# datastryio/weaviate

Measured on AMD Instinct MI355X. Metric: batched 10-NN QPS at recall@10≥0.95, 1M×128-d L2, on 1/2/4/8 MI355X, higher is better.
Workload: dtype f32 (f16 MFMA keys certified by an error bound, f32 reference-order re-rank); 1 GPU; exact brute-force 10-NN, 1,000,000 x 128-d l2-squared, 10000-query batch (BASELINE configs[1]); N=1000000, dim=128, nq=10000, k=10, metric=l2-squared, mode=exact, split=corpus, parallelism=corpus sharded over 1 GPU(s) by id range

## Files before the change

weaviate_amd/csrc/wv_api.hip:

```cpp
#include <hip/hip_runtime.h>
#include <hipcub/hipcub.hpp>

#include <algorithm>
#include <array>
#include <atomic>
#include <chrono>
#include <cmath>
#include <cstdio>
#include <cstdlib>
#include <condition_variable>
#include <cstring>
#include <mutex>
#include <string>
#include <thread>
#include <vector>

#include "../../include/wvgpu.h"
#include "wv_device.h"

#include "wv_params.h"

extern "C" {
hipError_t wv_launch_bf_mfma(const wv::BfParams* p, hipStream_t s);
hipError_t wv_launch_bf_finalize(const wv::BfFinParams* p, hipStream_t s);
hipError_t wv_launch_bf_finalize_wide(const wv::BfFinParams* p, hipStream_t s);
hipError_t wv_launch_exact_scan(const wv::ScanParams* p, hipStream_t s);
hipError_t wv_launch_fb(const wv::FbParams* p, hipStream_t s);
hipError_t wv_launch_fbd(const int32_t* flags, int nq, const wv::FbParams* fb, hipStream_t s);
hipError_t wv_launch_fbd_mark(const int32_t* status, int nq, int32_t* flags, float* thr, const float* out_d,
                              const int32_t* out_n, int k, hipStream_t s);
hipError_t wv_launch_hnsw_stats(const uint32_t* counters, int nq, unsigned long long* acc, hipStream_t s);
hipError_t wv_launch_rownorm(const float* X, uint64_t N, int D, int ldx, float* norm2, unsigned int* maxbits,
                             hipStream_t s);
hipError_t wv_launch_normalize(const float* in, float* out, uint64_t n, int D, int ld, hipStream_t s);
hipError_t wv_launch_scale(const float* in, float* out, uint64_t n, float scale, hipStream_t s);
hipError_t wv_launch_qnorm(const float* Q, int nq, int D, int ldq, int metric, float* out, float* absmax_part,
                           hipStream_t s);
hipError_t wv_launch_hnsw(const wv::HnswParams* p, int waves_per_block, hipStream_t s);
hipError_t wv_launch_hnsw_wg(const wv::HnswParams* p, hipStream_t s);
hipError_t wv_launch_build_search(const wv::BuildParams* b, int waves_per_block, hipStream_t s);
hipError_t wv_launch_build_select(const wv::BuildParams* b, hipStream_t s);
hipError_t wv_launch_build_link(const wv::BuildParams* b, hipStream_t s);
int wv_hnsw_per_wave_words(int dpad, int efc, int sc, int vc_log2, int xs_log2);
int wv_hnsw_side_per_wave_words(int dpad, int side_rows, int vc_log2, int xs_log2);
int wv_hnsw_reg_per_wave_words(int dpad, int vc_log2);
hipError_t wv_launch_hnsw_side(const wv::HnswParams* p, int waves_per_block, int ev, hipStream_t s);
hipError_t wv_launch_sbd_scan(const wv::SbdParams* p, hipStream_t s);
hipError_t wv_sbd_sort(unsigned long long* keys, unsigned long long* tmp, const unsigned int* cnt, int nq, int cap,
                       int* offsets, void** scratch, size_t* scratch_cap, hipStream_t s);
hipError_t wv_launch_pq_encode(const float* X, int ldx, const uint64_t* ids, uint64_t n_rows, const wv::PqParams* pq,
                               uint8_t* codes, hipStream_t s);
hipError_t wv_launch_pq_scan(const wv::PqScanParams* p, hipStream_t s);
hipError_t wv_launch_split_rows(const float* in, int ld_in, const uint64_t* ids, uint64_t n, uint64_t n_valid, int D,
                                float scale, void* out, int ld_out, uint64_t out_row0, hipStream_t s);
hipError_t wv_launch_h16_rows(const float* in, int ld_in, const uint64_t* ids, uint64_t n, int D, int ns, float sign,
                              float scale, const unsigned int* scale_from_max, void* out, uint64_t out_row0,
                              unsigned int* res_max_bits, float* res_out, int wide_layout, hipStream_t s);
hipError_t wv_launch_h16_rows_gather(const float* in, int ld_in, const uint32_t* gather, uint64_t n, uint64_t n_pad,
                                     int D, int ns, float scale, void* out, hipStream_t s);
hipError_t wv_launch_h16_compact_aux(const float* xnorm, const uint32_t* rowidx, uint64_t n, const uint32_t* n_dev,
                                     float* cxnorm, uint64_t* excl, uint64_t excl_words, hipStream_t s);
hipError_t wv_launch_remap_ids(uint32_t* ids, int nq, int n_slots, int per_slot, int bq, uint64_t ntiles,
                               uint64_t units_per_block, const uint32_t* rowidx, uint64_t n_rows, const uint32_t* n_dev,
                               hipStream_t s);
hipError_t wv_launch_absmax(const float* in, int ld, uint64_t n, int D, unsigned int* max_bits, hipStream_t s);
hipError_t wv_launch_h16_qscale(const float* part, int nparts, unsigned int* max_bits, float bsign, float* qscale,
                                hipStream_t s);
hipError_t wv_launch_h16_xns(const float* xnorm, uint64_t n, float sx, const float* qscale, float* xns, hipStream_t s);
hipError_t wv_launch_bf_h16(const wv::H16Params* p, int ns, int seed, hipStream_t s);
hipError_t wv_launch_bf_h16w(const wv::H16Params* p, hipStream_t s);
// ... 470 lines not shown
    return WV_OK;
}

int run_h16(wv_index* ix, const float* d_q, int nq, int k, const uint64_t* d_allow, uint64_t allow_nbits, uint64_t N,
            uint64_t* d_out_ids, float* d_out_d, int32_t* d_out_n, hipStream_t s, std::vector<int32_t>& fails,
            const uint32_t* rowidx = nullptr, const uint32_t* n_dev = nullptr) {
    const int ns = ix->h16_ns;
    const bool wd = ix->h16_wide;
    const int wg_per_cu = 1;
    const int tile_rows = wd ? wv::HW_BN : wv::H_BN, bq = wd ? wv::HW_BQ : 512;
    const int seed_prod = wd ? wv::HW_PROD : wv::H_PROD;
    const int prod = seed_prod;
    const int kp = wv::BF_KP;
    const uint64_t ntl = (N + tile_rows - 1) / tile_rows;
    const uint64_t words = ntl * (uint64_t)(tile_rows / 64);
    const uint64_t* allow = d_allow;
    if (d_allow && (allow_nbits + 63) / 64 < words) {
        HIP_TRY(ix->allow_pad.ensure(words * 8));
        HIP_TRY(hipMemsetAsync(ix->allow_pad.p, 0, words * 8, s));
        if (allow_nbits)
            HIP_TRY(hipMemcpyAsync(ix->allow_pad.p, d_allow, (allow_nbits + 63) / 64 * 8, hipMemcpyDeviceToDevice, s));
        allow = ix->allow_pad.as<uint64_t>();
    }
    const int nqb = (nq + bq - 1) / bq;
    const size_t qbytes = (size_t)nqb * bq * ns * 16 * 2;
    HIP_TRY(ix->qimg16.ensure(qbytes));
    HIP_TRY(ix->qres.ensure((size_t)nq * 4));
    HIP_TRY(ix->tau.ensure((size_t)nq * 4));
    HIP_TRY(ix->gtau.ensure((size_t)nq * 4));
    HIP_TRY(ix->q_nrm2.ensure((size_t)nq * 4));
    HIP_TRY(ix->fail.ensure((size_t)nq * 4));
    HIP_TRY(ix->fail_thr.ensure((size_t)nq * 4));
    const float bsign = ix->metric == WV_L2_SQUARED ? -2.f : -1.f;
    HIP_TRY(ix->qmax_part.ensure((size_t)((nq + 3) / 4) * 4));
    HIP_TRY(wv_launch_qnorm(d_q, nq, ix->dim, ix->dpad, ix->metric, ix->q_nrm2.as<float>(), ix->qmax_part.as<float>(),
                            s));
    HIP_TRY(hipMemsetAsync(ix->qimg16.p, 0, qbytes, s));
    HIP_TRY(wv_launch_h16_qscale(ix->qmax_part.as<float>(), (nq + 3) / 4, ix->qmax.as<unsigned int>(), bsign,
                                 ix->qscale.as<float>(), s));
    HIP_TRY(wv_launch_h16_rows(d_q, ix->dpad, nullptr, nq, ix->dim, ns, bsign, 1.f, ix->qmax.as<unsigned int>(),
                               ix->qimg16.p, 0, nullptr, ix->qres.as<float>(), 0, s));
    const void* ximg = ix->ximg16.p;
    const float* xnorm = ix->xnorm.as<float>();
    const uint64_t* excl = ix->excl.as<uint64_t>();
    if (rowidx) {
        const uint64_t rows = ntl * tile_rows, ew = rows / 64 + 2;
        HIP_TRY(ix->cxnorm.ensure(rows * 4));
        HIP_TRY(ix->cexcl.ensure(ew * 8));
        HIP_TRY(hipMemsetAsync(ix->cxnorm.p, 0, rows * 4, s));
        if (!wd) {
            const size_t ib = rows * (size_t)ns * 16 * 2;
            HIP_TRY(ix->cimg16.ensure(ib));
            HIP_TRY(wv_launch_h16_rows_gather(ix->vecs.as<float>(), ix->ldx, rowidx, N, rows, ix->dim, ns, ix->h16_sx,
                                              ix->cimg16.p, s));
            ximg = ix->cimg16.p;
        }
        HIP_TRY(wv_launch_h16_compact_aux(ix->xnorm.as<float>(), rowidx, N, n_dev, ix->cxnorm.as<float>(),
                                          ix->cexcl.as<uint64_t>(), ew, s));
        xnorm = ix->cxnorm.as<float>();
        excl = ix->cexcl.as<uint64_t>();
        allow = nullptr;
    }
    if (ix->metric == WV_L2_SQUARED)
        HIP_TRY(wv_launch_h16_xns(xnorm, ntl * tile_rows, ix->h16_sx, ix->qscale.as<float>(), ix->xns.as<float>(), s));
    wv::H16Params hp{};
    hp.X = ximg;
    hp.rowidx = wd ? rowidx : nullptr;
    hp.Q = ix->qimg16.p;
    hp.xns = ix->xns.as<float>();
    hp.excl = excl;
    hp.allow = allow;
    hp.qscale = ix->qscale.as<float>();
    hp.sx = ix->h16_sx;
    hp.N = N;
    hp.nq = nq;
    hp.metric = ix->metric;
    hp.n_qblocks = nqb;
    hp.wide_rows = 128;
    hp.clean_tiles = wd ? 0 : rowidx ? N / wv::H_BN : allow ? 0 : std::min<uint64_t>(ix->clean_words, N / wv::H_BN);
    hp.locality = 1;
    wv::BfFinParams fp{};
    fp.X = ix->vecs.as<float>();
    fp.Q = d_q;
    fp.qnorm = ix->q_nrm2.as<float>();
    fp.xnorm_max = ix->maxnorm_host;
    fp.nq = nq;
    fp.D = ix->dim;
    fp.ldx = ix->ldx;
    fp.ldq = ix->dpad;
    fp.metric = ix->metric;
    fp.k = k;
    fp.id_base = ix->cfg.id_base;
    fp.out_ids = d_out_ids;
    fp.out_d = d_out_d;
    fp.out_n = d_out_n;
    fp.fail = ix->fail.as<int32_t>();
    fp.fail_thr = ix->fail_thr.as<float>();
// ... 79 lines not shown
        sp.bq = bq;
        sp.prod = seed_prod;
        if (seed_lists) {
            HIP_TRY(wv_launch_h16_seed(&sp, s));
            HIP_TRY(ix->seed_d.ensure((size_t)nq * ss.n_slots * prod * kp * 4));
            HIP_TRY(ix->seed_id.ensure((size_t)nq * ss.n_slots * prod * kp * 4));
            hp.ntiles = ss.ntiles;
            hp.ntiles_real = ss.ntiles;
            hp.units_per_block = ss.units_per_block;
            hp.n_slots = ss.n_slots;
            hp.tile_stride = 1;
            hp.tile_base = ntl_main;
            hp.tau = ix->tau.as<float>();
            hp.out_d = ix->seed_d.as<float>();
            hp.out_id = ix->seed_id.as<uint32_t>();
            HIP_TRY(wv_launch_bf_h16(&hp, ns, 0, s));
            hp.tile_base = 0;
            hp.tau = nullptr;
            sp.minima = ix->seed_d.as<float>();
            sp.ids = ix->seed_id.as<uint32_t>();
            sp.n_slots = ss.n_slots;
            sp.ntiles = ss.ntiles;
            sp.units_per_block = ss.units_per_block;
            sp.prod = prod * kp;
            sp.out_d = ix->cand_d.as<float>();
            sp.out_id = ix->cand_id.as<uint32_t>();
            sp.out_slots = out_slots;
            sp.out_ntiles = sch.ntiles;
            sp.out_upb = sch.units_per_block;
        }
        HIP_TRY(wv_launch_h16_seed(&sp, s));
        return WV_OK;
    };
    if (seed) {
        TREC(6);
        int mult = 4;
        if (const char* e = std::getenv("WV_H16_LIST_MULT")) mult = std::max(1, std::atoi(e));
        if (int rc = seed_minima(seed_lists ? mult * sample : sample)) return rc;
        TREC(7);
    }
    hp.ntiles = sch.ntiles;
    hp.ntiles_real = ntl_main;
    hp.out_slots = seed_lists ? out_slots : 0;
    hp.units_per_block = sch.units_per_block;
    hp.n_slots = sch.n_slots;
    hp.n_dev = n_dev;
    hp.tile_stride = 1;
    hp.tau = nullptr;
    if (!seed) HIP_TRY(hipMemsetAsync(ix->gtau.p, 0xFF, (size_t)nq * 4, s));
    hp.gtau = ix->gtau.as<unsigned int>();
    hp.kth = k <= (wd ? 2 * kp : prod * kp) && !seed && !std::getenv("WV_H16_NO_RUNNING")
                 ? k
                 : 0;
    if (xs_fits(sch)) {
        const size_t gb = (size_t)nq * 2 * sch.n_slots * 4;
        HIP_TRY(ix->gslot.ensure(gb));
        HIP_TRY(hipMemsetAsync(ix->gslot.p, 0x7F, gb, s));
        hp.gslot = ix->gslot.as<float>();
        hp.xslot = 1;
        hp.kth = k;
    }
    if (hp.kth) {
        HIP_TRY(ix->marg.ensure((size_t)nq * 4));
        HIP_TRY(wv_launch_h16_margin(ix->metric, ix->dim, ix->q_nrm2.as<float>(), ix->qres.as<float>(),
                                     ix->maxnorm_host, ix->h16_ex, ix->h16_sx, ix->qscale.as<float>(), nq,
                                     ix->marg.as<float>(), s));
        hp.marg = ix->marg.as<float>();
    }
    hp.out_d = ix->cand_d.as<float>();
    hp.out_id = ix->cand_id.as<uint32_t>();
    const bool rotate = !wd && nqb >= 2 && sch.ntiles == ntl_main;
    if (rotate) hp.locality |= 2;
    if (int rc = block_order(ix, (uint64_t)nqb, sch, s, &hp.block_order, rotate)) return rc;
    TREC(0);
    HIP_TRY(wd ? wv_launch_bf_h16w(&hp, s) : wv_launch_bf_h16(&hp, ns, 0, s));
    TREC(1);
    if (rowidx && wide)
        HIP_TRY(wv_launch_remap_ids(ix->cand_id.as<uint32_t>(), nq, sch.n_slots, prod * kp, bq, sch.ntiles,
                                    sch.units_per_block, rowidx, N, n_dev, s));
    if (rowidx && !wide) {
        fp.rowidx = rowidx;
        fp.rowidx_n = N;
        fp.rowidx_ndev = n_dev;
    }
    fp.cand_d = ix->cand_d.as<float>();
    fp.cand_id = ix->cand_id.as<uint32_t>();
    fp.n_slots = out_slots;
    fp.extra_slot = seed_lists ? 1 : 0;
    fp.ntiles = sch.ntiles;
    fp.units_per_block = sch.units_per_block;
    HIP_TRY(wv_launch_h16_gtau(ix->gtau.as<unsigned int>(), nq, ix->h16_sx, ix->qscale.as<float>(), ix->tau.as<float>(),
                               s));
    fp.tau_in = ix->tau.as<float>();
    TREC(2);
    HIP_TRY(wide ? wv_launch_bf_finalize_wide(&fp, s) : wv_launch_bf_finalize(&fp, s));
    TREC(3);
    (void)fails;
    return WV_OK;
}

int queue_fbd(wv_index* ix, const float* d_q, int nq, int k, const uint64_t* d_allow, uint64_t allow_nbits,
              uint64_t allow_stride, uint64_t* d_out_ids, float* d_out_d, int32_t* d_out_n, hipStream_t s) {
    const uint64_t N = ix->n_rows;
    HIP_TRY(ix->fbd_list.ensure((size_t)nq * 4));
    HIP_TRY(ix->fbd_nf.ensure(16));
    HIP_TRY(ix->fbd_over.ensure((size_t)nq * 4));
    HIP_TRY(ix->fbd_cd.ensure((size_t)nq * wv::FB_CAP * 4));
    HIP_TRY(ix->fbd_ci.ensure((size_t)nq * wv::FB_CAP * 4));
    HIP_TRY(ix->fbd_cn.ensure((size_t)nq * 4));
    HIP_TRY(ix->fbd_scr.ensure((size_t)wv::FBD_SCR * std::max<uint64_t>(N, 1) * 4));
    HIP_TRY(ix->stat_acc.ensure(48));
    wv::FbParams bp{};
    bp.X = ix->vecs.as<float>();
    bp.Q = d_q;
    bp.qidx = ix->fbd_list.as<int32_t>();
    bp.thr = ix->fail_thr.as<float>();
    bp.tomb = ix->excl.as<uint64_t>();
    bp.tomb_nbits = ix->capacity;
    bp.allow = d_allow;
    bp.allow_nbits = allow_nbits;
    bp.allow_stride = allow_stride;
    bp.N = N;
    bp.nf = nq;
    bp.D = ix->dim;
    bp.ldx = ix->ldx;
    bp.ldq = ix->dpad;
// ... 2222 lines not shown
```

weaviate_amd/csrc/wv_bf.hip:

```cpp
#include "wv_device.h"
#include "wv_params.h"
#include "wv_topk.h"

#include <float.h>

namespace wv {


typedef __bf16 bf16x8 __attribute__((ext_vector_type(8)));




__device__ __forceinline__ void list_insert(float (&ld)[BF_KP], uint32_t (&li)[BF_KP], float d, uint32_t id) {
#pragma unroll
    for (int i = 0; i < BF_KP; ++i) {
        const bool lt = key_less(d, id, ld[i], li[i]);
        const float td = ld[i];
        const uint32_t ti = li[i];
        ld[i] = lt ? d : ld[i];
        li[i] = lt ? id : li[i];
        d = lt ? td : d;
        id = lt ? ti : id;
    }
// ... 599 lines not shown
                if (hi == mi && hd == md && mi != WV_NIL) head++;
                if (lane == 0) { sd[r] = md; si[r] = mi; }
            }
        }
    }
    __builtin_amdgcn_wave_barrier();
    {
        const float dk = sd[FIN_KF - 1];
        const uint32_t ik = si[FIN_KF - 1];
        if (key_less(dk, ik, bound, bound_id)) { bound = dk; bound_id = ik; }
    }
    if (p.h16 && bound != FLT_MAX) bound *= 1.0f / (p.sx * p.qscale[0]);
    if (p.tau_in) bound = fminf(bound, p.tau_in[q]);

    for (int i = lane; i < ((p.D + 3) & ~3); i += 64) qv[i] = i < p.D ? p.Q[(size_t)q * p.ldq + i] : 0.f;
    __builtin_amdgcn_wave_barrier();

    int n_sel = 0;
    for (int j = 0; j < FIN_KF; ++j) n_sel += (si[j] != WV_NIL);
    __builtin_amdgcn_wave_barrier();
    if (p.rowidx) {
        const uint64_t nr = p.rowidx_ndev ? (uint64_t)*p.rowidx_ndev : p.rowidx_n;
        uint32_t v = WV_NIL;
        if (lane < FIN_KF && si[lane] != WV_NIL && si[lane] < nr) v = p.rowidx[si[lane]];
        const uint64_t vm = __ballot(v != WV_NIL);
        __builtin_amdgcn_wave_barrier();
        if (lane < FIN_KF) si[lane] = WV_NIL;
        __builtin_amdgcn_wave_barrier();
        if (v != WV_NIL) si[mbcnt64(vm)] = v;
        n_sel = __popcll(vm);
        if (lane < FIN_KF && lane >= n_sel) sd[lane] = FLT_MAX;
        __builtin_amdgcn_wave_barrier();
    }
    exact_dist_rows<METRIC, FIN_KF / 8>(qv, p.X, p.ldx, p.D, si, n_sel, sd, lane);
    __builtin_amdgcn_wave_barrier();
    float myd = FLT_MAX;
    uint32_t myi = WV_NIL;
    int rank = 0;
    if (lane < FIN_KF) {
        myd = sd[lane];
        myi = si[lane];
        const uint64_t mykey = fin_key(myd, myi);
        for (int j = 0; j < FIN_KF; ++j)
            rank += fin_key(sd[j], si[j]) < mykey;
    }
    __builtin_amdgcn_wave_barrier();
    const int k = p.k;
    int nvalid = 0;
    for (int j = 0; j < FIN_KF; ++j) nvalid += (si[j] != WV_NIL);
    if (lane < FIN_KF && myi != WV_NIL && rank < k && !p.tau_out) {
        p.out_ids[(size_t)q * k + rank] = p.id_base + myi;
        p.out_d[(size_t)q * k + rank] = myd;
    }
    float dk = -FLT_MAX;
    const int nk = nvalid < k ? nvalid : k;
    if (lane < FIN_KF && myi != WV_NIL && rank == nk - 1) dk = myd;
    for (int m = 32; m >= 1; m >>= 1) dk = fmaxf(dk, __shfl_xor(dk, m, 64));

    const float u = 5.9604645e-08f;
    const float D4 = (float)(p.D + 4);
    float eps, bfull;
    const float acc_f = p.split ? 12.f : 4.f;
    const float split_e = p.split ? 4.f * 1.52587890625e-05f : 0.f;
    if (METRIC == WV_METRIC_L2) {
        const float qn = sqrtf(p.qnorm[q]);
        const float s = qn + p.xnorm_max;
        eps = acc_f * D4 * u * s * s + 2.f * split_e * qn * p.xnorm_max;
        bfull = bound + p.qnorm[q];
    } else {
        const float qn = p.qnorm[q];
        eps = acc_f * D4 * u * qn * p.xnorm_max + 4.f * u + split_e * qn * p.xnorm_max;
        bfull = METRIC == WV_METRIC_DOT ? bound : 1.0f + bound;
    }
    eps *= 1.0001f;
    if (p.h16) eps = h16_eps(METRIC, p.D, p.qnorm[q], p.xnorm_max, p.ex_max, p.qres[q]);
    if (p.tau_out) {
        float tau = __builtin_inff();
        if (nvalid >= k && dk < FLT_MAX) {
            const float off = METRIC == WV_METRIC_L2 ? p.qnorm[q] : (METRIC == WV_METRIC_DOT ? 0.f : 1.0f);
            tau = dk - off + eps;
            tau += 4.f * u * (fabsf(dk) + fabsf(off) + eps) + 1e-3f * eps;
        }
        if (lane == 0) p.tau_out[q] = tau;
        return;
    }
    bool certified;
    if (nvalid < k) certified = bound == FLT_MAX;
    else certified = (bound == FLT_MAX) || (bfull - eps > dk);
    if (lane == 0) {
        p.out_n[q] = nk;
        p.fail[q] = certified ? 0 : 1;
        p.fail_thr[q] = nvalid < k ? __builtin_inff() : dk;
    }
}

template <bool FAST>
__global__ __launch_bounds__(64) void wv_bf_finalize_kernel(BfFinParams p) {
    extern __shared__ float qv[];
    const int dpad = (p.D + 3) & ~3;
    float* sd = qv + dpad;
    uint32_t* si = reinterpret_cast<uint32_t*>(sd + FIN_KF);
    float* kept_d = reinterpret_cast<float*>(si + FIN_KF);
    uint32_t* kept_i = reinterpret_cast<uint32_t*>(kept_d + 256);
    const int q = blockIdx.x;
    if (q >= p.nq) return;
    if (p.metric == WV_METRIC_L2) finalize_one<WV_METRIC_L2, FAST>(p, q, sd, si, qv, kept_d, kept_i);
    else if (p.metric == WV_METRIC_DOT) finalize_one<WV_METRIC_DOT, FAST>(p, q, sd, si, qv, kept_d, kept_i);
    else finalize_one<WV_METRIC_COSINE, FAST>(p, q, sd, si, qv, kept_d, kept_i);
// ... 530 lines not shown
    }
    if (norm == 0.f) {
        for (int i = 0; i < D; ++i) o[i] = 0.f;
        return;
    }
    const float nn = (float)sqrt((double)norm);
    for (int i = 0; i < D; ++i) o[i] = __fdiv_rn(v[i], nn);
}

__device__ __forceinline__ uint16_t bf16_rn(float v) {
    const uint32_t b = __float_as_uint(v);
    return (uint16_t)((b + 0x7FFFu + ((b >> 16) & 1u)) >> 16);
}
__global__ void wv_split_rows_kernel(const float* in, int ld_in, const uint64_t* ids, uint64_t n, uint64_t n_valid,
                                     int D, float scale, uint16_t* out, int ld_out, uint64_t out_row0) {
    const uint64_t t = (uint64_t)blockIdx.x * blockDim.x + threadIdx.x;
    const uint64_t r = t / (uint64_t)ld_out;
    const int k = (int)(t % (uint64_t)ld_out);
    if (r >= n) return;
    const uint64_t row = ids ? ids[r] : r;
    const float v = (k < D && r < n_valid) ? scale * in[row * ld_in + k] : 0.f;
    const uint16_t hi = bf16_rn(v);
    const uint16_t lo = bf16_rn(v - __uint_as_float((uint32_t)hi << 16));
    const uint64_t o = split_hi_index(out_row0 + row, k, ld_out / BF_BK);
    out[o] = hi;
    out[o + 512] = lo;
}

__global__ void wv_scale_rows_kernel(const float* in, float* out, uint64_t n, float s) {
    const uint64_t i = (uint64_t)blockIdx.x * blockDim.x + threadIdx.x;
    if (i < n) out[i] = s * in[i];
}

__global__ __launch_bounds__(256) void wv_qnorm_kernel(const float* Q, int nq, int D, int ldq, int metric, float* out,
                                                       float* absmax_part) {
    __shared__ float wmax[4];
    const int lane = threadIdx.x & 63, w = threadIdx.x >> 6;
    const int r = blockIdx.x * 4 + w;
    float s = 0.f, m = 0.f;
    if (r < nq) {
        const float* q = Q + (size_t)r * ldq;
        for (int i = lane; i < D; i += 64) {
            const float v = q[i];
            s = __builtin_fmaf(v, v, s);
            m = fmaxf(m, fabsf(v));
        }
    }
    for (int o = 32; o >= 1; o >>= 1) {
        s += __shfl_xor(s, o, 64);
        m = fmaxf(m, __shfl_xor(m, o, 64));
    }
    if (r < nq && lane == 0) out[r] = metric == WV_METRIC_L2 ? s : sqrtf(s * (1.0f + 1e-6f)) * (1.0f + 1e-6f);
    if (absmax_part) {
        if (lane == 0) wmax[w] = m;
        __syncthreads();
        if (threadIdx.x == 0) absmax_part[blockIdx.x] = fmaxf(fmaxf(wmax[0], wmax[1]), fmaxf(wmax[2], wmax[3]));
    }
}

}

extern "C" {

hipError_t wv_launch_bf_mfma(const wv::BfParams* p, hipStream_t s) {
    if (p->X == nullptr || p->Q == nullptr) return hipErrorInvalidValue;
    const uint64_t total = (uint64_t)p->n_qblocks * p->ntiles;
    const unsigned nb = (unsigned)((total + p->units_per_block - 1) / p->units_per_block);
    if (nb == 0) return hipSuccess;
    if (p->split) {
        const int nk = p->ldx / wv::BF_BK;
        if (p->ldx % wv::BF_BK || p->ldq != p->ldx || nk < 1 || nk > 4 || p->rowidx || p->allow_stride)
            return hipErrorInvalidValue;
        const bool l2 = p->metric == WV_METRIC_L2;
        const bool wide = p->bq == 2 * wv::BF_BQ;
        if (!wide && p->bq != wv::BF_BQ) return hipErrorInvalidValue;
        const size_t lds = (size_t)nk * (wide ? 32768 : 16384) + (wide ? 8 : 4) * 256;
#define WV_SPLIT_LAUNCH(NK)                                                                                   \
        if (wide) {                                                                                           \
            if (l2) hipLaunchKernelGGL((wv::wv_bf_split_kernel<NK, true, 4>), dim3(nb), dim3(512), lds, s, *p);  \
            else hipLaunchKernelGGL((wv::wv_bf_split_kernel<NK, false, 4>), dim3(nb), dim3(512), lds, s, *p);    \
        } else {                                                                                              \
            if (l2) hipLaunchKernelGGL((wv::wv_bf_split_kernel<NK, true, 2>), dim3(nb), dim3(256), lds, s, *p);  \
            else hipLaunchKernelGGL((wv::wv_bf_split_kernel<NK, false, 2>), dim3(nb), dim3(256), lds, s, *p);    \
        }
        switch (nk) {
// ... 95 lines not shown
hipError_t wv_launch_exact_scan(const wv::ScanParams* p, hipStream_t s) {
    uint64_t blocks = (p->N + 31) / 32;
    if (blocks > 8192) blocks = 8192;
    if (blocks == 0) blocks = 1;
    hipLaunchKernelGGL(wv::wv_exact_scan_kernel, dim3((unsigned)blocks), dim3(256), p->D * sizeof(float), s, *p);
    return hipGetLastError();
}

hipError_t wv_launch_rownorm(const float* X, uint64_t N, int D, int ldx, float* norm2, unsigned int* maxbits,
                             hipStream_t s) {
    if (N == 0) return hipSuccess;
    hipLaunchKernelGGL(wv::wv_rownorm_kernel, dim3((unsigned)((N + 255) / 256)), dim3(256), 0, s, X, N, D, ldx,
                       norm2, maxbits);
    return hipGetLastError();
}

hipError_t wv_launch_normalize(const float* in, float* out, uint64_t n, int D, int ld, hipStream_t s) {
    if (n == 0) return hipSuccess;
    hipLaunchKernelGGL(wv::wv_normalize_kernel, dim3((unsigned)((n + 255) / 256)), dim3(256), 0, s, in, out, n, D,
                       ld);
    return hipGetLastError();
}

hipError_t wv_launch_scale(const float* in, float* out, uint64_t n, float scale, hipStream_t s) {
    if (n == 0) return hipSuccess;
    hipLaunchKernelGGL(wv::wv_scale_rows_kernel, dim3((unsigned)((n + 255) / 256)), dim3(256), 0, s, in, out, n,
                       scale);
    return hipGetLastError();
}

hipError_t wv_launch_qnorm(const float* Q, int nq, int D, int ldq, int metric, float* out, float* absmax_part,
                           hipStream_t s) {
    if (nq == 0) return hipSuccess;
    hipLaunchKernelGGL(wv::wv_qnorm_kernel, dim3((nq + 3) / 4), dim3(256), 0, s, Q, nq, D, ldq, metric, out,
                       absmax_part);
    return hipGetLastError();
}

}
```

weaviate_amd/csrc/wv_h16.hip:

```cpp
#include "wv_device.h"
#include "wv_params.h"
#include "wv_topk.h"

#include <float.h>

#include "wv_h16_dev.h"

namespace wv {


constexpr bool min_steps_cover(int ns) {
    unsigned m = 0;
    for (int k = 0; k < ns; ++k) {
        if (k == 0) m |= 7u;
        else if (k <= 6) m |= 3u << (2 * k + 1);
        if (k == ns - 1)
            for (int r = ns <= 7 ? 2 * ns + 1 : 15; r < 16; ++r) m |= 1u << r;
    }
    return m == 0xFFFFu;
}

template <int NS, bool L2, bool SEED, bool XS = false>
__global__ __launch_bounds__(512, 1) void wv_bf_h16_kernel(H16Params p) {
    static_assert(min_steps_cover(NS), "the spread tile minima must cover all 16 keys of a half");
// ... 800 lines not shown
                    const float th = fminf(ld[BF_KP - 1], pt);
                    const float m = min16(A);
                    const bool x = m <= th;
                    if (__any(x)) {
                        WV_DBG_COUNT(3)
                        min_extract(m, x, A, pt, ld, li, rr);
                    }
                };
                xt(A0, l0d, l0i, pt0, rb);
                xt(B0, l0d, l0i, pt0, rb + 32);
                xt(A1, l1d, l1i, pt1, rb);
                xt(B1, l1d, l1i, pt1, rb + 32);
#endif
            }
            if (running && (tc < 8 || (tc & 3) == 3)) publish();
        }
        vm_wait(0);
        block_barrier();
        const int prod = rh * 2 + khalf;
        const size_t per_q = (size_t)p.n_slots * HW_PROD * BF_KP;
        if (jq0 < p.nq) {
            const size_t base = (size_t)jq0 * per_q + ((size_t)slot * HW_PROD + prod) * BF_KP;
#pragma unroll
            for (int i = 0; i < BF_KP; ++i) { p.out_d[base + i] = l0d[i]; p.out_id[base + i] = l0i[i]; }
        }
        if (jq1 < p.nq) {
            const size_t base = (size_t)jq1 * per_q + ((size_t)slot * HW_PROD + prod) * BF_KP;
#pragma unroll
            for (int i = 0; i < BF_KP; ++i) { p.out_d[base + i] = l1d[i]; p.out_id[base + i] = l1i[i]; }
        }
    }
}

__global__ __launch_bounds__(64) void wv_h16_seed_kernel(H16SeedParams p) {
    const int q = blockIdx.x;
    const int lane = threadIdx.x;
    if (q >= p.nq) return;
    const int prod = p.prod ? p.prod : H_PROD;
    const int n = bf_slots_of((uint64_t)(q / p.bq), p.ntiles, p.units_per_block) * prod;
    const float* m = p.minima + (size_t)q * p.n_slots * prod;
    const float inv_s = 1.0f / (p.sx * p.qscale[0]);
    float mk = __builtin_inff();
    if (p.ids) {
        const size_t off = (size_t)q * p.n_slots * prod;
        uint64_t kk[4];
#pragma unroll
        for (int j = 0; j < 4; ++j) {
            const int e = 64 * j + lane;
            const uint32_t id = e < n ? p.ids[off + e] : WV_NIL;
            kk[j] = fin_key(id != WV_NIL ? p.minima[off + e] : FLT_MAX, id);
        }
        bitonic256_wave(kk, lane);
        float d;
        uint32_t id;
        fin_unkey(kk[0], d, id);
        const float dk = __shfl(d, p.k - 1, 64);
        const uint32_t ik = (uint32_t)__shfl((int)id, p.k - 1, 64);
        if (ik != WV_NIL) mk = dk;
        const int os = bf_slots_of((uint64_t)(q / p.bq), p.out_ntiles, p.out_upb);
        const size_t ob = ((size_t)q * p.out_slots + os) * H_PROD * BF_KP;
        if (lane < H_PROD * BF_KP) {
            const size_t o = ob + (size_t)(lane & 1) * BF_KP + (lane >> 1);
            p.out_d[o] = d;
            p.out_id[o] = id;
        }
    } else if (n <= 256) {
        float v[4];
#pragma unroll
        for (int j = 0; j < 4; ++j) v[j] = 64 * j + lane < n ? m[64 * j + lane] : __builtin_inff();
#pragma unroll
        for (int kk = 2; kk <= 256; kk <<= 1) {
#pragma unroll
            for (int jj = kk >> 1; jj > 0; jj >>= 1) {
                if (jj >= 64) {
                    const int mm = jj >> 6;
#pragma unroll
                    for (int j = 0; j < 4; ++j) {
                        const int pj = j ^ mm;
                        if (pj <= j) continue;
                        const bool up = ((64 * j + lane) & kk) == 0;
                        const float lo = fminf(v[j], v[pj]), hi = fmaxf(v[j], v[pj]);
                        v[j] = up ? lo : hi;
                        v[pj] = up ? hi : lo;
                    }
                } else {
                    const bool lower = (lane & jj) == 0;
#pragma unroll
                    for (int j = 0; j < 4; ++j) {
                        const float o = __shfl_xor(v[j], jj, 64);
                        const bool up = ((64 * j + lane) & kk) == 0;
                        v[j] = (lower == up) ? fminf(v[j], o) : fmaxf(v[j], o);
                    }
                }
            }
        }
        const int e = p.k - 1;
        float sel = v[0];
#pragma unroll
// ... 86 lines not shown
}

__global__ void wv_absmax_kernel(const float* in, int ld, uint64_t n, int D, unsigned int* max_bits) {
    const uint64_t i = (uint64_t)blockIdx.x * blockDim.x + threadIdx.x;
    float m = 0.f;
    for (uint64_t j = i; j < n * (uint64_t)D; j += (uint64_t)gridDim.x * blockDim.x) {
        const uint64_t r = j / (uint64_t)D, c = j % (uint64_t)D;
        m = fmaxf(m, fabsf(in[r * ld + c]));
    }
    for (int s = 32; s >= 1; s >>= 1) m = fmaxf(m, __shfl_xor(m, s, 64));
    if ((threadIdx.x & 63) == 0) atomicMax(max_bits, __float_as_uint(m));
}

__global__ __launch_bounds__(256) void wv_h16_qscale_kernel(const float* part, int nparts, unsigned int* max_bits,
                                                            float bsign, float* qscale) {
    __shared__ float wm[4];
    float m = 0.f;
    if (part)
        for (int i = threadIdx.x; i < nparts; i += blockDim.x) m = fmaxf(m, part[i]);
    for (int o = 32; o >= 1; o >>= 1) m = fmaxf(m, __shfl_xor(m, o, 64));
    if ((threadIdx.x & 63) == 0) wm[threadIdx.x >> 6] = m;
    __syncthreads();
    if (threadIdx.x == 0) {
        float mx = part ? fmaxf(fmaxf(wm[0], wm[1]), fmaxf(wm[2], wm[3])) : __uint_as_float(*max_bits);
        if (part) *max_bits = __float_as_uint(mx);
        qscale[0] = pow2_scale_for(mx * fabsf(bsign));
    }
}
__global__ void wv_h16_xns_kernel(const float* xnorm, uint64_t n, float sx, const float* qscale, float* xns) {
    const uint64_t i = (uint64_t)blockIdx.x * blockDim.x + threadIdx.x;
    if (i < n) xns[i] = xnorm[i] * (sx * qscale[0]);
}

}

extern "C" {

float wv_h16_pow2_scale(float maxabs) {
    if (!(maxabs > 0.f) || !(maxabs < FLT_MAX)) return 1.f;
    int e;
    frexpf(maxabs, &e);
    e = 14 - e;
    e = e > 100 ? 100 : (e < -100 ? -100 : e);
    return ldexpf(1.f, e);
}

hipError_t wv_launch_h16_rows(const float* in, int ld_in, const uint64_t* ids, uint64_t n, int D, int ns, float sign,
                              float scale, const unsigned int* scale_from_max, void* out, uint64_t out_row0,
                              unsigned int* res_max_bits, float* res_out, int wide_layout, hipStream_t s) {
    if (n == 0) return hipSuccess;
    if (ns < 1 || ns > wv::HW_NS_MAX || D > ns * 16) return hipErrorInvalidValue;
    hipLaunchKernelGGL(wv::wv_h16_rows_kernel, dim3((unsigned)((n + 3) / 4)), dim3(256), 0, s, in, ld_in, ids,
                       (const uint32_t*)nullptr, n, D, ns, sign, scale, scale_from_max, static_cast<uint16_t*>(out),
                       out_row0, res_max_bits, res_out, wide_layout);
    return hipGetLastError();
}

__global__ void wv_h16_img_gather_kernel(const float* __restrict__ in, int ld_in, const uint32_t* __restrict__ gather,
                                         uint64_t n, uint64_t n_pad, int D, int ns, float scale, uint4* __restrict__ out) {
    const uint64_t i = (uint64_t)blockIdx.x * blockDim.x + threadIdx.x;
    const uint64_t total = n_pad / 32 * (uint64_t)ns * 64;
    if (i >= total) return;
    const uint64_t block = i >> 6;
    const int lane = (int)(i & 63);
    const uint64_t grp = block / (uint64_t)ns;
    const int step = (int)(block - grp * ns);
// ... 66 lines not shown
                              n_dev, cxnorm);
    hipLaunchKernelGGL(wv_excl_tail_kernel, dim3((unsigned)((excl_words + 255) / 256)), dim3(256), 0, s, excl, n,
                       n_dev, excl_words);
    return hipGetLastError();
}

hipError_t wv_launch_remap_ids(uint32_t* ids, int nq, int n_slots, int per_slot, int bq, uint64_t ntiles,
                               uint64_t units_per_block, const uint32_t* rowidx, uint64_t n_rows, const uint32_t* n_dev,
                               hipStream_t s) {
    if (nq == 0) return hipSuccess;
    hipLaunchKernelGGL(wv_remap_ids_kernel, dim3((unsigned)nq), dim3(64), 0, s, ids, nq, n_slots, per_slot, bq, ntiles,
                       units_per_block, rowidx, n_rows, n_dev);
    return hipGetLastError();
}

hipError_t wv_launch_absmax(const float* in, int ld, uint64_t n, int D, unsigned int* max_bits, hipStream_t s) {
    if (n == 0) return hipSuccess;
    uint64_t blocks = (n * (uint64_t)D + 255) / 256;
    if (blocks > 1024) blocks = 1024;
    hipLaunchKernelGGL(wv::wv_absmax_kernel, dim3((unsigned)blocks), dim3(256), 0, s, in, ld, n, D, max_bits);
    return hipGetLastError();
}

hipError_t wv_launch_h16_qscale(const float* part, int nparts, unsigned int* max_bits, float bsign, float* qscale,
                                hipStream_t s) {
    hipLaunchKernelGGL(wv::wv_h16_qscale_kernel, dim3(1), dim3(256), 0, s, part, nparts, max_bits, bsign, qscale);
    return hipGetLastError();
}

hipError_t wv_launch_h16_xns(const float* xnorm, uint64_t n, float sx, const float* qscale, float* xns, hipStream_t s) {
    if (n == 0) return hipSuccess;
    hipLaunchKernelGGL(wv::wv_h16_xns_kernel, dim3((unsigned)((n + 255) / 256)), dim3(256), 0, s, xnorm, n, sx, qscale,
                       xns);
    return hipGetLastError();
}

hipError_t wv_launch_bf_h16(const wv::H16Params* p, int ns, int seed, hipStream_t s) {
    const uint64_t total = (uint64_t)p->n_qblocks * p->ntiles;
    const unsigned nb = (unsigned)((total + p->units_per_block - 1) / p->units_per_block);
    if (nb == 0) return hipSuccess;
    if (ns < 1 || ns > wv::H_NS_MAX || !p->X || !p->Q || !p->excl || !p->qscale || p->tile_stride < 1 ||
        (p->out_slots && p->out_slots < p->n_slots) || (seed && (p->out_slots || p->tile_base)))
        return hipErrorInvalidValue;
    const bool l2 = p->metric == WV_METRIC_L2;
    if (l2 && !p->xns) return hipErrorInvalidValue;
    const size_t lds = (size_t)wv::H_STAGES * wv::H_TPS8 * (2 * ns * 64 + 17) * 16 +
                       (!seed && p->xslot ? (size_t)wv::H_XS_LDS : 0);
    if (!seed && p->xslot && (!p->gtau || !p->gslot || !p->marg || p->kth < 1)) return hipErrorInvalidValue;
#define WV_H16_GO(NS, L, S)                                                                                    \
    if (!S && p->xslot)                                                                                        \
        hipLaunchKernelGGL((wv::wv_bf_h16_kernel<NS, L, false, true>), dim3(nb), dim3(512), lds, s, *p);       \
    else hipLaunchKernelGGL((wv::wv_bf_h16_kernel<NS, L, S>), dim3(nb), dim3(512), lds, s, *p);
#define WV_H16_LAUNCH(NS)                     \
    if (seed) {                               \
        if (l2) { WV_H16_GO(NS, true, true) } \
        else { WV_H16_GO(NS, false, true) }   \
    } else {                                  \
        if (l2) { WV_H16_GO(NS, true, false) } \
        else { WV_H16_GO(NS, false, false) }  \
    }
    switch (ns) {
        case 1: WV_H16_LAUNCH(1) break;
        case 2: WV_H16_LAUNCH(2) break;
        case 3: WV_H16_LAUNCH(3) break;
        case 4: WV_H16_LAUNCH(4) break;
        case 5: WV_H16_LAUNCH(5) break;
// ... 14 lines not shown
    return hipGetLastError();
}

hipError_t wv_launch_h16_gtau(const unsigned int* gtau, int nq, float sx, const float* qscale, float* tau,
                              hipStream_t s) {
    if (nq == 0) return hipSuccess;
    hipLaunchKernelGGL(wv::wv_h16_gtau_kernel, dim3((nq + 255) / 256), dim3(256), 0, s, gtau, nq, sx, qscale, tau);
    return hipGetLastError();
}

hipError_t wv_launch_bf_h16w(const wv::H16Params* p, hipStream_t s) {
    const uint64_t total = (uint64_t)p->n_qblocks * p->ntiles;
    const unsigned nb = (unsigned)((total + p->units_per_block - 1) / p->units_per_block);
    if (nb == 0) return hipSuccess;
    if (p->ns < 2 * wv::HW_KC || p->ns > wv::HW_NS_MAX || p->ns % wv::HW_KC || !p->X || !p->Q || !p->excl ||
        p->tile_stride != 1 || p->tile_base != 0 || p->out_slots != 0)
        return hipErrorInvalidValue;
    const bool l2 = p->metric == WV_METRIC_L2;
    if (l2 && !p->xns) return hipErrorInvalidValue;
    if (p->wide_rows != 128) return hipErrorInvalidValue;
    using St = wv::HWStage<128>;
    const size_t lds = ((size_t)wv::HW_STAGES * St::U4 + 2 * St::EX_U4) * 16 + 8 * 256 + 2 * 8 * 2 * 256;
    if (l2) hipLaunchKernelGGL((wv::wv_bf_h16w_kernel<true, 128>), dim3(nb), dim3(512), lds, s, *p);
    else hipLaunchKernelGGL((wv::wv_bf_h16w_kernel<false, 128>), dim3(nb), dim3(512), lds, s, *p);
    return hipGetLastError();
}

hipError_t wv_launch_h16_seed(const wv::H16SeedParams* p, hipStream_t s) {
    if (p->nq == 0) return hipSuccess;
    if (p->k < 1 || p->k > wv::BF_WIDE_KMAX) return hipErrorInvalidValue;
    if (p->ids && (p->k > 64 || p->prod != wv::H_PROD * wv::BF_KP || (size_t)p->n_slots * p->prod > 256 ||
                   !p->out_d || !p->out_id || p->out_slots < 1))
        return hipErrorInvalidValue;
    hipLaunchKernelGGL(wv::wv_h16_seed_kernel, dim3(p->nq), dim3(64), 0, s, *p);
    return hipGetLastError();
}

}
```

weaviate_amd/csrc/wv_params.h:

```cpp
#pragma once
#include <stdint.h>

namespace wv {

constexpr int BF_BQ = 128;
constexpr int BF_BN = 128;
constexpr int BF_BK = 32;
constexpr int BF_LDT = 36;
constexpr int BF_KP = 8;
constexpr int BF_PROD = 4;
constexpr int FIN_KF = 32;
constexpr int BF_FAST_KMAX = 32;
constexpr int BF_WIDE_KMAX = 256;
constexpr int FINW_NE = 8192;
constexpr int FINW_KF = 1024;
constexpr int HNSW_EF_MAX = 512;

struct BfParams {
    const float* X;
    const float* Q;
    const float* xnorm;
    const uint64_t* tomb;
    const uint64_t* allow;
    const uint32_t* rowidx;
// ... 116 lines not shown
    const float* marg;
    float* gslot;
    int xslot;
    int ns;
    int wide_rows;
    const uint32_t* rowidx;
    const uint32_t* n_dev;
};

constexpr int HW_BN = 256;
constexpr int HW_BQ = 256;
constexpr int HW_KC = 4;
constexpr int HW_PROD = 4;
constexpr int HW_NS_MAX = 64;

#if defined(__HIPCC__)
__host__ __device__
#endif
inline unsigned int h16_key_enc(float f) {
    union { float f; unsigned int u; } v;
    v.f = f;
    return (v.u & 0x80000000u) ? ~v.u : (v.u | 0x80000000u);
}
#if defined(__HIPCC__)
__host__ __device__
#endif
inline float h16_key_dec(unsigned int k) {
    if (k >= 0xFF800000u) return __builtin_inff();
    union { float f; unsigned int u; } v;
    v.u = (k & 0x80000000u) ? (k & 0x7FFFFFFFu) : ~k;
    return v.f;
}

struct H16SeedParams {
    const float* minima;
    int n_slots;
    uint64_t ntiles, units_per_block;
    int nq, k, metric, D;
    const float* qscale;
    float sx;
    const float* qnorm;
    float xnorm_max, ex_max;
    const float* qres;
    float* tau;
    unsigned int* gtau;
    int bq;
    int prod;
    const uint32_t* ids;
    float* out_d;
    uint32_t* out_id;
    int out_slots;
    uint64_t out_ntiles, out_upb;
};

struct BfFinParams {
    const float* X;
    const float* Q;
    const float* cand_d;
    const uint32_t* cand_id;
    const float* qnorm;
    float xnorm_max;
    int n_slots;
    int extra_slot;
    uint64_t ntiles, units_per_block;
    int nq, D, ldx, ldq, metric, k;
    uint64_t id_base;
    uint64_t* out_ids;
    float* out_d;
    int32_t* out_n;
    int32_t* fail;
    float* fail_thr;
    int split;
    int bq;
    int prod;
    int kp;
    int finw_ne;
    int h16;
    const float* qscale;
    float sx;
    float ex_max;
    const float* qres;
    const float* tau_in;
    float* tau_out;
    const uint32_t* rowidx;
    uint64_t rowidx_n;
    const uint32_t* rowidx_ndev;
};

constexpr int FB_CAP = 2048;
struct FbParams {
    const float* X;
    const float* Q;
    const int32_t* qidx;
    const float* thr;
    const uint64_t* tomb;
    const uint64_t* allow;
    uint64_t tomb_nbits, allow_nbits, allow_stride;
    uint64_t N;
    int nf, D, ldx, ldq, metric, k;
    uint64_t id_base;
    float* cand_d;
    uint32_t* cand_id;
    uint32_t* cand_n;
    uint64_t* out_ids;
    float* out_d;
    int32_t* out_n;
    int32_t* overflow;
    const int32_t* d_nf;
    float* scratch;
    int n_scr;
    unsigned long long* fb_total;
};
constexpr int FBD_SCR = 8;

struct ScanParams {
// ... 126 lines not shown
```

Baseline: 4.292 million queries/s.

## Fuse h16 query prologue into one kernel and limit finalize re-rank

Several small pre-scan launches are merged into one prologue kernel: the memset, qscale, query f16 image build, xns scaling, gslot init and margin. The qnorm kernel now handles 16 rows per block, and the seed kernel packs four queries per block with a shuffle-rank path for up to 64 candidates. The finalize step re-ranks in f32 only the candidates within a 3*eps band of the k-th key, tightening the bound with the first excluded one. This cuts launch overhead and exact distance work, but correctness depends on the error bound holding, and the bound is recomputed in the prologue.

```diff
diff --git a/weaviate_amd/csrc/wv_api.hip b/weaviate_amd/csrc/wv_api.hip
--- a/weaviate_amd/csrc/wv_api.hip
+++ b/weaviate_amd/csrc/wv_api.hip
@@ -36,6 +36,9 @@
 hipError_t wv_launch_scale(const float* in, float* out, uint64_t n, float scale, hipStream_t s);
 hipError_t wv_launch_qnorm(const float* Q, int nq, int D, int ldq, int metric, float* out, float* absmax_part,
                            hipStream_t s);
+hipError_t wv_launch_qnorm_coarse(const float* Q, int nq, int D, int ldq, int metric, float* out, float* absmax_part,
+                                  hipStream_t s);
+hipError_t wv_launch_h16_prologue(const wv::H16PrologueParams* p, hipStream_t s);
 hipError_t wv_launch_hnsw(const wv::HnswParams* p, int waves_per_block, hipStream_t s);
 hipError_t wv_launch_hnsw_wg(const wv::HnswParams* p, hipStream_t s);
 hipError_t wv_launch_build_search(const wv::BuildParams* b, int waves_per_block, hipStream_t s);
@@ -572,14 +575,10 @@
     HIP_TRY(ix->fail.ensure((size_t)nq * 4));
     HIP_TRY(ix->fail_thr.ensure((size_t)nq * 4));
     const float bsign = ix->metric == WV_L2_SQUARED ? -2.f : -1.f;
-    HIP_TRY(ix->qmax_part.ensure((size_t)((nq + 3) / 4) * 4));
-    HIP_TRY(wv_launch_qnorm(d_q, nq, ix->dim, ix->dpad, ix->metric, ix->q_nrm2.as<float>(), ix->qmax_part.as<float>(),
-                            s));
-    HIP_TRY(hipMemsetAsync(ix->qimg16.p, 0, qbytes, s));
-    HIP_TRY(wv_launch_h16_qscale(ix->qmax_part.as<float>(), (nq + 3) / 4, ix->qmax.as<unsigned int>(), bsign,
-                                 ix->qscale.as<float>(), s));
-    HIP_TRY(wv_launch_h16_rows(d_q, ix->dpad, nullptr, nq, ix->dim, ns, bsign, 1.f, ix->qmax.as<unsigned int>(),
-                               ix->qimg16.p, 0, nullptr, ix->qres.as<float>(), 0, s));
+    const int nparts = (nq + wv::QNORM_COARSE - 1) / wv::QNORM_COARSE;
+    HIP_TRY(ix->qmax_part.ensure((size_t)nparts * 4));
+    HIP_TRY(wv_launch_qnorm_coarse(d_q, nq, ix->dim, ix->dpad, ix->metric, ix->q_nrm2.as<float>(),
+                                   ix->qmax_part.as<float>(), s));
     const void* ximg = ix->ximg16.p;
     const float* xnorm = ix->xnorm.as<float>();
     const uint64_t* excl = ix->excl.as<uint64_t>();
@@ -601,8 +600,6 @@
         excl = ix->cexcl.as<uint64_t>();
         allow = nullptr;
     }
-    if (ix->metric == WV_L2_SQUARED)
-        HIP_TRY(wv_launch_h16_xns(xnorm, ntl * tile_rows, ix->h16_sx, ix->qscale.as<float>(), ix->xns.as<float>(), s));
     wv::H16Params hp{};
     hp.X = ximg;
     hp.rowidx = wd ? rowidx : nullptr;
@@ -748,6 +745,44 @@
         HIP_TRY(wv_launch_h16_seed(&sp, s));
         return WV_OK;
     };
+    int kth = k <= (wd ? 2 * kp : prod * kp) && !seed && !std::getenv("WV_H16_NO_RUNNING") ? k : 0;
+    const bool xslot = xs_fits(sch);
+    const size_t gslot_words = xslot ? (size_t)nq * 2 * sch.n_slots : 0;
+    if (xslot) {
+        HIP_TRY(ix->gslot.ensure(gslot_words * 4));
+        kth = k;
+    }
+    if (kth) HIP_TRY(ix->marg.ensure((size_t)nq * 4));
+    {
+        wv::H16PrologueParams pp{};
+        pp.Q = d_q;
+        pp.ldq = ix->dpad;
+        pp.nq = nq;
+        pp.D = ix->dim;
+        pp.ns = ns;
+        pp.metric = ix->metric;
+        pp.bsign = bsign;
+        pp.part = ix->qmax_part.as<float>();
+        pp.nparts = nparts;
+        pp.qmax = ix->qmax.as<unsigned int>();
+        pp.qscale = ix->qscale.as<float>();
+        pp.qimg = ix->qimg16.p;
+        pp.img_rows = nqb * bq;
+        pp.qres = ix->qres.as<float>();
+        pp.qnorm = ix->q_nrm2.as<float>();
+        pp.xnorm_max = ix->maxnorm_host;
+        pp.ex_max = ix->h16_ex;
+        pp.sx = ix->h16_sx;
+        pp.marg = kth ? ix->marg.as<float>() : nullptr;
+        if (ix->metric == WV_L2_SQUARED) {
+            pp.xnorm = xnorm;
+            pp.xns = ix->xns.as<float>();
+            pp.n_xns = ntl * tile_rows;
+        }
+        pp.gslot = xslot ? ix->gslot.as<float>() : nullptr;
+        pp.n_gslot = gslot_words;
+        HIP_TRY(wv_launch_h16_prologue(&pp, s));
+    }
     if (seed) {
         TREC(6);
         int mult = 4;
@@ -765,24 +800,12 @@
     hp.tau = nullptr;
     if (!seed) HIP_TRY(hipMemsetAsync(ix->gtau.p, 0xFF, (size_t)nq * 4, s));
     hp.gtau = ix->gtau.as<unsigned int>();
-    hp.kth = k <= (wd ? 2 * kp : prod * kp) && !seed && !std::getenv("WV_H16_NO_RUNNING")
-                 ? k
-                 : 0;
-    if (xs_fits(sch)) {
-        const size_t gb = (size_t)nq * 2 * sch.n_slots * 4;
-        HIP_TRY(ix->gslot.ensure(gb));
-        HIP_TRY(hipMemsetAsync(ix->gslot.p, 0x7F, gb, s));
+    hp.kth = kth;
+    if (xslot) {
         hp.gslot = ix->gslot.as<float>();
         hp.xslot = 1;
-        hp.kth = k;
-    }
-    if (hp.kth) {
-        HIP_TRY(ix->marg.ensure((size_t)nq * 4));
-        HIP_TRY(wv_launch_h16_margin(ix->metric, ix->dim, ix->q_nrm2.as<float>(), ix->qres.as<float>(),
-                                     ix->maxnorm_host, ix->h16_ex, ix->h16_sx, ix->qscale.as<float>(), nq,
-                                     ix->marg.as<float>(), s));
-        hp.marg = ix->marg.as<float>();
-    }
+    }
+    if (kth) hp.marg = ix->marg.as<float>();
     hp.out_d = ix->cand_d.as<float>();
     hp.out_id = ix->cand_id.as<uint32_t>();
     const bool rotate = !wd && nqb >= 2 && sch.ntiles == ntl_main;
@@ -808,6 +831,8 @@
     HIP_TRY(wv_launch_h16_gtau(ix->gtau.as<unsigned int>(), nq, ix->h16_sx, ix->qscale.as<float>(), ix->tau.as<float>(),
                                s));
     fp.tau_in = ix->tau.as<float>();
+    const char* ra = std::getenv("WV_FIN_RERANK_ALL");
+    fp.rerank_limit = ra && std::atoi(ra) != 0 ? 0 : 1;
     TREC(2);
     HIP_TRY(wide ? wv_launch_bf_finalize_wide(&fp, s) : wv_launch_bf_finalize(&fp, s));
     TREC(3);
diff --git a/weaviate_amd/csrc/wv_bf.hip b/weaviate_amd/csrc/wv_bf.hip
--- a/weaviate_amd/csrc/wv_bf.hip
+++ b/weaviate_amd/csrc/wv_bf.hip
@@ -655,7 +655,36 @@
         if (lane < FIN_KF && lane >= n_sel) sd[lane] = FLT_MAX;
         __builtin_amdgcn_wave_barrier();
     }
-    exact_dist_rows<METRIC, FIN_KF / 8>(qv, p.X, p.ldx, p.D, si, n_sel, sd, lane);
+    const float u = 5.9604645e-08f;
+    const float D4 = (float)(p.D + 4);
+    float eps;
+    const float acc_f = p.split ? 12.f : 4.f;
+    const float split_e = p.split ? 4.f * 1.52587890625e-05f : 0.f;
+    if (METRIC == WV_METRIC_L2) {
+        const float qn = sqrtf(p.qnorm[q]);
+        const float s = qn + p.xnorm_max;
+        eps = acc_f * D4 * u * s * s + 2.f * split_e * qn * p.xnorm_max;
+    } else {
+        const float qn = p.qnorm[q];
+        eps = acc_f * D4 * u * qn * p.xnorm_max + 4.f * u + split_e * qn * p.xnorm_max;
+    }
+    eps *= 1.0001f;
+    if (p.h16) eps = h16_eps(METRIC, p.D, p.qnorm[q], p.xnorm_max, p.ex_max, p.qres[q]);
+    int kf = n_sel;
+    if (p.rerank_limit && !p.tau_out) {
+        const float ks = p.h16 ? p.sx * p.qscale[0] : 1.f;
+        const int kk = p.k < FIN_KF ? p.k : FIN_KF;
+        const float lim = sd[kk - 1] + 3.f * eps * ks * 1.001f;
+        const uint64_t in = __ballot(lane < n_sel && sd[lane] <= lim);
+        kf = in ? 64 - __clzll(in) : 0;
+        const int kmin = kk < n_sel ? kk : n_sel;
+        kf = kf > kmin ? kf : kmin;
+        if (kf < FIN_KF && sd[kf] != FLT_MAX) bound = fminf(bound, p.h16 ? sd[kf] * (1.0f / ks) : sd[kf]);
+        __builtin_amdgcn_wave_barrier();
+        if (lane >= kf && lane < FIN_KF) { sd[lane] = FLT_MAX; si[lane] = WV_NIL; }
+        __builtin_amdgcn_wave_barrier();
+    }
+    exact_dist_rows<METRIC, FIN_KF / 8>(qv, p.X, p.ldx, p.D, si, kf, sd, lane);
     __builtin_amdgcn_wave_barrier();
     float myd = FLT_MAX;
     uint32_t myi = WV_NIL;
@@ -680,23 +709,9 @@
     if (lane < FIN_KF && myi != WV_NIL && rank == nk - 1) dk = myd;
     for (int m = 32; m >= 1; m >>= 1) dk = fmaxf(dk, __shfl_xor(dk, m, 64));
 
-    const float u = 5.9604645e-08f;
-    const float D4 = (float)(p.D + 4);
-    float eps, bfull;
-    const float acc_f = p.split ? 12.f : 4.f;
-    const float split_e = p.split ? 4.f * 1.52587890625e-05f : 0.f;
-    if (METRIC == WV_METRIC_L2) {
-        const float qn = sqrtf(p.qnorm[q]);
-        const float s = qn + p.xnorm_max;
-        eps = acc_f * D4 * u * s * s + 2.f * split_e * qn * p.xnorm_max;
-        bfull = bound + p.qnorm[q];
-    } else {
-        const float qn = p.qnorm[q];
-        eps = acc_f * D4 * u * qn * p.xnorm_max + 4.f * u + split_e * qn * p.xnorm_max;
-        bfull = METRIC == WV_METRIC_DOT ? bound : 1.0f + bound;
-    }
-    eps *= 1.0001f;
-    if (p.h16) eps = h16_eps(METRIC, p.D, p.qnorm[q], p.xnorm_max, p.ex_max, p.qres[q]);
+    float bfull;
+    if (METRIC == WV_METRIC_L2) bfull = bound + p.qnorm[q];
+    else bfull = METRIC == WV_METRIC_DOT ? bound : 1.0f + bound;
     if (p.tau_out) {
         float tau = __builtin_inff();
         if (nvalid >= k && dk < FLT_MAX) {
@@ -1293,25 +1308,33 @@
     if (i < n) out[i] = s * in[i];
 }
 
+template <int RPW>
 __global__ __launch_bounds__(256) void wv_qnorm_kernel(const float* Q, int nq, int D, int ldq, int metric, float* out,
                                                        float* absmax_part) {
     __shared__ float wmax[4];
     const int lane = threadIdx.x & 63, w = threadIdx.x >> 6;
-    const int r = blockIdx.x * 4 + w;
-    float s = 0.f, m = 0.f;
-    if (r < nq) {
-        const float* q = Q + (size_t)r * ldq;
-        for (int i = lane; i < D; i += 64) {
-            const float v = q[i];
-            s = __builtin_fmaf(v, v, s);
+    const int r0 = (blockIdx.x * 4 + w) * RPW;
+    float s[RPW], m = 0.f;
+#pragma unroll
+    for (int j = 0; j < RPW; ++j) s[j] = 0.f;
+    for (int i = lane; i < D; i += 64) {
+#pragma unroll
+        for (int j = 0; j < RPW; ++j) {
+            if (r0 + j >= nq) continue;
+            const float v = Q[(size_t)(r0 + j) * ldq + i];
+            s[j] = __builtin_fmaf(v, v, s[j]);
             m = fmaxf(m, fabsf(v));
         }
     }
     for (int o = 32; o >= 1; o >>= 1) {
-        s += __shfl_xor(s, o, 64);
+#pragma unroll
+        for (int j = 0; j < RPW; ++j) s[j] += __shfl_xor(s[j], o, 64);
         m = fmaxf(m, __shfl_xor(m, o, 64));
     }
-    if (r < nq && lane == 0) out[r] = metric == WV_METRIC_L2 ? s : sqrtf(s * (1.0f + 1e-6f)) * (1.0f + 1e-6f);
+#pragma unroll
+    for (int j = 0; j < RPW; ++j)
+        if (r0 + j < nq && lane == 0)
+            out[r0 + j] = metric == WV_METRIC_L2 ? s[j] : sqrtf(s[j] * (1.0f + 1e-6f)) * (1.0f + 1e-6f);
     if (absmax_part) {
         if (lane == 0) wmax[w] = m;
         __syncthreads();
@@ -1473,9 +1496,18 @@
 hipError_t wv_launch_qnorm(const float* Q, int nq, int D, int ldq, int metric, float* out, float* absmax_part,
                            hipStream_t s) {
     if (nq == 0) return hipSuccess;
-    hipLaunchKernelGGL(wv::wv_qnorm_kernel, dim3((nq + 3) / 4), dim3(256), 0, s, Q, nq, D, ldq, metric, out,
+    hipLaunchKernelGGL(wv::wv_qnorm_kernel<1>, dim3((nq + 3) / 4), dim3(256), 0, s, Q, nq, D, ldq, metric, out,
                        absmax_part);
     return hipGetLastError();
 }
 
-}
+hipError_t wv_launch_qnorm_coarse(const float* Q, int nq, int D, int ldq, int metric, float* out, float* absmax_part,
+                                  hipStream_t s) {
+    if (nq == 0) return hipSuccess;
+    static_assert(wv::QNORM_COARSE % 4 == 0, "four waves per block");
+    hipLaunchKernelGGL(wv::wv_qnorm_kernel<wv::QNORM_COARSE / 4>, dim3((nq + wv::QNORM_COARSE - 1) / wv::QNORM_COARSE),
+                       dim3(256), 0, s, Q, nq, D, ldq, metric, out, absmax_part);
+    return hipGetLastError();
+}
+
+}
diff --git a/weaviate_amd/csrc/wv_h16.hip b/weaviate_amd/csrc/wv_h16.hip
--- a/weaviate_amd/csrc/wv_h16.hip
+++ b/weaviate_amd/csrc/wv_h16.hip
@@ -856,9 +856,9 @@
     }
 }
 
-__global__ __launch_bounds__(64) void wv_h16_seed_kernel(H16SeedParams p) {
-    const int q = blockIdx.x;
-    const int lane = threadIdx.x;
+__global__ __launch_bounds__(256) void wv_h16_seed_kernel(H16SeedParams p) {
+    const int q = blockIdx.x * 4 + (threadIdx.x >> 6);
+    const int lane = threadIdx.x & 63;
     if (q >= p.nq) return;
     const int prod = p.prod ? p.prod : H_PROD;
     const int n = bf_slots_of((uint64_t)(q / p.bq), p.ntiles, p.units_per_block) * prod;
@@ -888,6 +888,15 @@
             p.out_d[o] = d;
             p.out_id[o] = id;
         }
+    } else if (n <= 64) {
+        const float v = lane < n ? m[lane] : __builtin_inff();
+        int rank = 0;
+        for (int j = 0; j < n; ++j) {
+            const float o = __shfl(v, j, 64);
+            rank += (o < v || (o == v && j < lane)) ? 1 : 0;
+        }
+        const uint64_t hit = __ballot(lane < n && rank == p.k - 1);
+        if (hit) mk = __shfl(v, __ffsll((unsigned long long)hit) - 1, 64);
     } else if (n <= 256) {
         float v[4];
 #pragma unroll
@@ -1040,6 +1049,65 @@
     if (i < n) xns[i] = xnorm[i] * (sx * qscale[0]);
 }
 
+__global__ __launch_bounds__(256) void wv_h16_prologue_kernel(H16PrologueParams p) {
+    const unsigned row_blocks = (unsigned)((p.img_rows + 3) / 4);
+    const unsigned xns_blocks = p.xns ? (unsigned)((p.n_xns + 1023) / 1024) : 0u;
+    const unsigned b = blockIdx.x;
+    if (b >= row_blocks + xns_blocks) {
+        const uint64_t i0 = (uint64_t)(b - row_blocks - xns_blocks) * 1024 + threadIdx.x;
+        uint32_t* g = reinterpret_cast<uint32_t*>(p.gslot);
+#pragma unroll
+        for (int j = 0; j < 4; ++j)
+            if (i0 + 256 * j < p.n_gslot) g[i0 + 256 * j] = 0x7F7F7F7Fu;
+        return;
+    }
+    __shared__ float wm[4];
+    float m = 0.f;
+    for (int i = threadIdx.x; i < p.nparts; i += 256) m = fmaxf(m, p.part[i]);
+    for (int o = 32; o >= 1; o >>= 1) m = fmaxf(m, __shfl_xor(m, o, 64));
+    if ((threadIdx.x & 63) == 0) wm[threadIdx.x >> 6] = m;
+    __syncthreads();
+    const float mx = fmaxf(fmaxf(wm[0], wm[1]), fmaxf(wm[2], wm[3]));
+    const float scale = pow2_scale_for(mx * fabsf(p.bsign));
+    if (b == 0 && threadIdx.x == 0) {
+        *p.qmax = __float_as_uint(mx);
+        p.qscale[0] = scale;
+    }
+    if (b >= row_blocks) {
+        const uint64_t i0 = (uint64_t)(b - row_blocks) * 1024 + threadIdx.x;
+#pragma unroll
+        for (int j = 0; j < 4; ++j)
+            if (i0 + 256 * j < p.n_xns) p.xns[i0 + 256 * j] = p.xnorm[i0 + 256 * j] * (p.sx * scale);
+        return;
+    }
+    const int r = (int)b * 4 + (int)(threadIdx.x >> 6);
+    const int lane = threadIdx.x & 63;
+    if (r >= p.img_rows) return;
+    uint16_t* out = static_cast<uint16_t*>(p.qimg);
+    if (r >= p.nq) {
+        for (int c = lane; c < p.ns * 2; c += 64)
+            *reinterpret_cast<uint4*>(out + h16_index((uint64_t)r, 8 * c, p.ns)) = make_uint4(0u, 0u, 0u, 0u);
+        return;
+    }
+    const int kmax = p.ns * 16;
+    float acc = 0.f;
+    for (int k = lane; k < kmax; k += 64) {
+        const float x = k < p.D ? p.bsign * p.Q[(uint64_t)r * (uint64_t)p.ldq + k] : 0.f;
+        const _Float16 h = (_Float16)(scale * x);
+        const float back = (float)h / scale;
+        const float e = x - back;
+        acc = __builtin_fmaf(e, e, acc);
+        out[h16_index((uint64_t)r, k, p.ns)] = __builtin_bit_cast(uint16_t, h);
+    }
+    for (int o = 32; o >= 1; o >>= 1) acc += __shfl_xor(acc, o, 64);
+    if (lane == 0) {
+        const float res = acc == 0.f ? 0.f : sqrtf(acc * (1.0f + 2e-5f)) * (1.0f + 1e-6f) + 1e-30f;
+        p.qres[r] = res;
+        if (p.marg)
+            p.marg[r] = 2.f * (p.sx * scale) * h16_eps(p.metric, p.D, p.qnorm[r], p.xnorm_max, p.ex_max, res) * 1.001f;
+    }
+}
+
 }
 
 extern "C" {
@@ -1172,6 +1240,18 @@
     if (n == 0) return hipSuccess;
     hipLaunchKernelGGL(wv::wv_h16_xns_kernel, dim3((unsigned)((n + 255) / 256)), dim3(256), 0, s, xnorm, n, sx, qscale,
                        xns);
+    return hipGetLastError();
+}
+
+hipError_t wv_launch_h16_prologue(const wv::H16PrologueParams* p, hipStream_t s) {
+    if (p->nq < 1 || p->img_rows < p->nq || p->img_rows % 32 || p->ns < 1 || p->ns > wv::HW_NS_MAX ||
+        p->D > p->ns * 16 || !p->Q || !p->part || p->nparts < 1 || !p->qmax || !p->qscale || !p->qimg || !p->qres ||
+        !p->qnorm || (p->xns && !p->xnorm) || (p->gslot ? p->n_gslot == 0 : p->n_gslot != 0))
+        return hipErrorInvalidValue;
+    const uint64_t nb = (uint64_t)(p->img_rows + 3) / 4 + (p->xns ? (p->n_xns + 1023) / 1024 : 0) +
+                        (p->n_gslot + 1023) / 1024;
+    if (nb > 0x7FFFFFFFull) return hipErrorInvalidValue;
+    hipLaunchKernelGGL(wv::wv_h16_prologue_kernel, dim3((unsigned)nb), dim3(256), 0, s, *p);
     return hipGetLastError();
 }
 
@@ -1252,7 +1332,7 @@
     if (p->ids && (p->k > 64 || p->prod != wv::H_PROD * wv::BF_KP || (size_t)p->n_slots * p->prod > 256 ||
                    !p->out_d || !p->out_id || p->out_slots < 1))
         return hipErrorInvalidValue;
-    hipLaunchKernelGGL(wv::wv_h16_seed_kernel, dim3(p->nq), dim3(64), 0, s, *p);
+    hipLaunchKernelGGL(wv::wv_h16_seed_kernel, dim3((p->nq + 3) / 4), dim3(256), 0, s, *p);
     return hipGetLastError();
 }
 
diff --git a/weaviate_amd/csrc/wv_params.h b/weaviate_amd/csrc/wv_params.h
--- a/weaviate_amd/csrc/wv_params.h
+++ b/weaviate_amd/csrc/wv_params.h
@@ -172,6 +172,29 @@
     return v.f;
 }
 
+constexpr int QNORM_COARSE = 16;
+
+struct H16PrologueParams {
+    const float* Q;
+    int ldq, nq, D, ns, metric;
+    float bsign;
+    const float* part;
+    int nparts;
+    unsigned int* qmax;
+    float* qscale;
+    void* qimg;
+    int img_rows;
+    float* qres;
+    const float* qnorm;
+    float xnorm_max, ex_max, sx;
+    float* marg;
+    const float* xnorm;
+    float* xns;
+    uint64_t n_xns;
+    float* gslot;
+    uint64_t n_gslot;
+};
+
 struct H16SeedParams {
     const float* minima;
     int n_slots;
@@ -221,6 +244,7 @@
     float ex_max;
     const float* qres;
     const float* tau_in;
+    int rerank_limit;
     float* tau_out;
     const uint32_t* rowidx;
     uint64_t rowidx_n;
```

New measurement: 4.345 million queries/s (median of 6 runs). 1.01x the previous value.
